# naver-ai/egtr

Measured on AMD Instinct MI355X. Metric: images/sec end-to-end SGG, 600x1000 input, N=200 queries, higher is better.
Workload: dtype f32; 1 GPU; VG inference: ResNet-50, N=200, 6 enc/6 dec, 150 classes, 50 predicates, 600x1000, bs=1/GPU fp32 (BASELINE configs[1]); hip_graph=True, gemm_tuning=True, miopen_find=True, parallelism=replicas x1 (independent images, no collective)

## Files before the change

egtr_amd/_lib.py:

```python
import ctypes
import os

import torch

_HERE = os.path.dirname(os.path.abspath(__file__))
LIB_PATH = os.environ.get("EGTR_HIP_LIBRARY") or os.path.join(_HERE, "libegtr_hip.so")

_P = ctypes.c_void_p
_I = ctypes.c_int
ABI_VERSION = 5

SIGNATURES = {
    "egtr_abi_version": [],
    "egtr_status_string": [_I],
    "egtr_last_hip_error": [],
    "egtr_msda_forward_f32": [_P, _P, _P, _P, _P, _P, _I, _I, _I, _I, _I, _I, _I, _P],
    "egtr_msda_forward_fused_vbias_f32": [_P, _P, _P, _P, _P, _P, _P, _I, _I, _I, _I, _I, _I, _I, _P, _P, _I, _I, _P, _P,
                                          _P],
    "egtr_msda_forward_fused_box_f32": [_P, _P, _P, _P, _P, _P, _P, _I, _I, _I, _I, _I, _I, _I, _P, _P, _I, _I, _P, _P,
                                        _P],
    "egtr_msda_backward_f32": [_P, _P, _P, _P, _P, _P, _P, _I, _I, _I, _I, _I, _I, _I, _P, _P, _P],
    "egtr_msda_backward_out_f32": [_P, _P, _P, _P, _P, _P, _P, _I, _I, _I, _I, _I, _I, _I, _P, _P, _P],
    "egtr_msda_forward_f64": [_P, _P, _P, _P, _P, _P, _I, _I, _I, _I, _I, _I, _I, _P],
    "egtr_msda_backward_f64": [_P, _P, _P, _P, _P, _P, _P, _I, _I, _I, _I, _I, _I, _I, _P, _P, _P],
# ... 18 lines not shown
    "egtr_bias_act_nhwc_bf16": [_P, _P, _P, _P, _P, ctypes.c_longlong, _I, _I],
    "egtr_bias_act_nhwc_f32": [_P, _P, _P, _P, _P, ctypes.c_longlong, _I, _I],
    "egtr_add_layernorm_bf16": [_P, _P, _P, _P, _P, _P, _I, _I, ctypes.c_float],
    "egtr_add_layernorm_pos_bf16": [_P, _P, _P, _P, _P, _P, _I, _I, ctypes.c_float, _P, _I, _P],
    "egtr_add_layernorm_f32": [_P, _P, _P, _P, _P, _P, _I, _I, ctypes.c_float],
    "egtr_sine_pos_embed_f32": [_P, _P, _P, _P, _P, _I, _I, _I, _I, ctypes.c_float, ctypes.c_float],
    "egtr_level_geometry_f32": [_P, _P, _I, _P, _P, _P, _I, _I, _I, _I, _I, ctypes.c_float, ctypes.c_float, _P, _P, _P,
                                _P, _P],
    "egtr_level_geometry_bf16": [_P, _P, _I, _P, _P, _P, _I, _I, _I, _I, _I, ctypes.c_float, ctypes.c_float, _P, _P, _P,
                                 _P, _P],
    "egtr_input_proj_groupnorm_flatten_f32": [_P, _I, _P, _P, _P, _P, _P, _I, _I, _I, ctypes.c_float, _P, _P],
    "egtr_input_proj_groupnorm_flatten_bf16": [_P, _I, _P, _P, _P, _P, _P, _I, _I, _I, ctypes.c_float, _P, _P],
    "egtr_input_proj_groupnorm_tokens_bf16": [_P, _I, _P, _P, _P, _P, _P, _I, _I, _I, ctypes.c_float, _P, _P],
    "egtr_input_proj_groupnorm_tokens_f32": [_P, _I, _P, _P, _P, _P, _P, _I, _I, _I, ctypes.c_float, _P, _P],
    "egtr_input_proj_groupnorm_tokens_workspace_floats": [_I, _P, _I],
    "egtr_bbox_overlaps_f64": [_P, _P, _P, _I, _I, _I, _P],
    "egtr_sgg_eval_width": [_I, _I],
    "egtr_sgg_eval_f32": [_P, _P, _I, _P, _P, _P, _I, _I, _I, _I, _P, _P, ctypes.c_longlong, _P, _P, _P, ctypes.c_longlong,
                          _P, _I, ctypes.c_double, _P, _P, _P],
    "egtr_sgg_zero_shot_f64": [_P, _P, _P, _P, ctypes.c_longlong, _P, _P, ctypes.c_longlong, _I, _I, _I, _I, _P, _P, _I, _P,
                               _P],
    "egtr_sgg_eval_phrdet_f32": [_P, _P, _I, _P, _P, _P, _I, _I, _I, _I, _P, _P, ctypes.c_longlong, _P, _P, _P,
                                 ctypes.c_longlong, _P, _I, ctypes.c_double, _P, _P, _P],
    "egtr_sgg_eval_preddet_f32": [_P, _P, _P, _I, _I, _I, _P, _P, ctypes.c_longlong, _P, ctypes.c_longlong, _P, _I, _P, _P,
                                  _P, _P, _P],
    "egtr_matched_topk_workspace_bytes": [_I, _I, _I],
    "egtr_matched_topk_f32": [_P, _P, _P, _P, _P, _I, _I, _I, _I, _I, _I, _P, _P, _P, _P, _P],
    "egtr_rel_stats_i64": [_P, _P, _P, ctypes.c_longlong, _P, _P, ctypes.c_longlong, _I, _I, _I, _P, _P],
    "egtr_rel_seen_bits_i64": [_P, _P, ctypes.c_longlong, _P],
    "egtr_oi_eval_width": [_I, _I],
# ... 66 lines not shown
    "egtr_proj_ln_x6_f32": [_P, _P, _I, _P, _P, _P, _I, _P, _P, ctypes.c_float, _P, _I, _P, _P, _I, _I],
    "egtr_proj_multi_x6_f32": [_P, _P, _I, _P, _P, _P, _I, _I, _I],
    "egtr_xs_bytes": [_I, _I],
    "egtr_xs_split_f32": [_P, _P, _I, _P, _I, _I, _I, _P, _P, _I],
    "egtr_rel_head_forward_bf16x6_f32": [_P] * 16 + [_I] * 6 + [_P] * 3 + [_I],
    "egtr_rel_head_forward_bf16x6_save_f32": [_P] * 16 + [_I] * 6 + [_P] * 5,
    "egtr_rel_head_streams_f32": [_P] * 4 + [_I] * 2 + [_P] * 3,
    "egtr_rel_head_forward_save_f32": [_P] * 16 + [_I] * 6 + [_P] * 5,
    "egtr_rel_head_backward_pairs_f32": [_P] * 6 + [_I] * 4 + [_P] * 5,
    "egtr_decoder_layer_f32": [_P, _P],
    "egtr_decoder_layer_workspace": [_I, _I, _P, _P, _P],
}
_RESTYPES = {"egtr_status_string": ctypes.c_char_p, "egtr_last_hip_error": ctypes.c_char_p,
             "egtr_ffn_packed_weights_bytes": ctypes.c_longlong,
             "egtr_input_proj_groupnorm_tokens_workspace_floats": ctypes.c_longlong,
             "egtr_msda_backward_bf16_workspace_floats": ctypes.c_longlong,
             "egtr_hungarian_match_scratch_doubles": ctypes.c_longlong,
             "egtr_relation_loss_workspace_bytes": ctypes.c_longlong,
             "egtr_column_sum_workspace_floats": ctypes.c_longlong,
             "egtr_add_layernorm_backward_workspace_floats": ctypes.c_longlong,
             "egtr_linear_split_bf16_wgrad_workspace_floats": ctypes.c_longlong,
             "egtr_dropout_add_layernorm_backward_workspace_floats": ctypes.c_longlong,
             "egtr_xs_bytes": ctypes.c_longlong, "egtr_sgg_eval_width": ctypes.c_longlong,
             "egtr_oi_eval_width": ctypes.c_longlong, "egtr_matched_topk_workspace_bytes": ctypes.c_longlong, "egtr_oi_select_workspace_bytes": ctypes.c_longlong}

_lib = None


class EgtrHipError(RuntimeError):
    pass
# ... 72 lines not shown
```

egtr_amd/csrc/elementwise.hip:

```cpp
#include <hip/hip_runtime.h>
#include <stdint.h>

#include "common.h"

namespace {

__global__ __launch_bounds__(256) void bias_act_nchw_vec4(const float* __restrict__ x, const float* __restrict__ bias,
                                                          const float* __restrict__ res, float* __restrict__ y,
                                                          long long n4, int C, int HW4, int relu) {
  for (long long i = blockIdx.x * (long long)blockDim.x + threadIdx.x; i < n4; i += (long long)gridDim.x * blockDim.x) {
    const int c = (int)((i / HW4) % C);
    const float b = bias[c];
    float4 v = reinterpret_cast<const float4*>(x)[i];
    v.x += b; v.y += b; v.z += b; v.w += b;
    if (res != nullptr) {
      const float4 r = reinterpret_cast<const float4*>(res)[i];
      v.x += r.x; v.y += r.y; v.z += r.z; v.w += r.w;
    }
    if (relu) { v.x = egtr_relu(v.x); v.y = egtr_relu(v.y); v.z = egtr_relu(v.z); v.w = egtr_relu(v.w); }
    reinterpret_cast<float4*>(y)[i] = v;
  }
}

__global__ __launch_bounds__(256) void bias_act_nchw_flat4(const float* __restrict__ x, const float* __restrict__ bias,
// ... 753 lines not shown
  const float* beta[4];
  int hw[4], start[4];
  long long chunk0[5];
  int cchunk0[5];
};

namespace {
__device__ __forceinline__ void load_group8(const unsigned short* x, size_t idx, float (&f)[8]) {
  unpack8(reinterpret_cast<const uint4*>(x)[idx], f);
}
__device__ __forceinline__ void load_group8(const float* x, size_t idx, float (&f)[8]) {
  const float4 a = reinterpret_cast<const float4*>(x)[2 * idx], b = reinterpret_cast<const float4*>(x)[2 * idx + 1];
  f[0] = a.x; f[1] = a.y; f[2] = a.z; f[3] = a.w; f[4] = b.x; f[5] = b.y; f[6] = b.z; f[7] = b.w;
}
constexpr int kGnTokChunk = 256;
template <typename T>
__global__ __launch_bounds__(256) void gn_partial_tokens(GnTokLevels P, int L, int chunks_total, double2* __restrict__ partial) {
  __shared__ double s_red[2][32][9];
  const int b = blockIdx.y;
  int l = 0;
  while (l + 1 < L && (int)blockIdx.x >= P.cchunk0[l + 1]) ++l;
  const int t_begin = ((int)blockIdx.x - P.cchunk0[l]) * kGnTokChunk, hw = P.hw[l];
  const int g = threadIdx.x & 31, ph = threadIdx.x >> 5;
  const T* x = static_cast<const T*>(P.x[l]) + (size_t)b * hw * 256;
  const float4 ba = *reinterpret_cast<const float4*>(P.conv_bias[l] + 8 * g), bb = *reinterpret_cast<const float4*>(P.conv_bias[l] + 8 * g + 4);
  const float cb[8] = {ba.x, ba.y, ba.z, ba.w, bb.x, bb.y, bb.z, bb.w};
  float s1 = 0.f, s2 = 0.f;
#pragma unroll
  for (int u0 = 0; u0 < kGnTokChunk / 8; u0 += 8) {
    float f[8][8];
#pragma unroll
    for (int u = 0; u < 8; ++u) {
      const int t = t_begin + ph + 8 * (u0 + u);
      if (t < hw) load_group8(x, (size_t)t * 32 + g, f[u]);
    }
#pragma unroll
    for (int u = 0; u < 8; ++u) {
      const int t = t_begin + ph + 8 * (u0 + u);
      if (t < hw) {
#pragma unroll
        for (int k = 0; k < 8; ++k) {
          const float v = f[u][k] + cb[k];
          s1 += v;
          s2 += v * v;
        }
      }
    }
  }
  s_red[0][g][ph] = (double)s1;
  s_red[1][g][ph] = (double)s2;
  __syncthreads();
  if (threadIdx.x < 32) {
    double t1 = 0.0, t2 = 0.0;
    for (int w = 0; w < 8; ++w) {
      t1 += s_red[0][threadIdx.x][w];
      t2 += s_red[1][threadIdx.x][w];
    }
    partial[((size_t)b * chunks_total + blockIdx.x) * 32 + threadIdx.x] = make_double2(t1, t2);
  }
// ... 53 lines not shown
#pragma unroll
    for (int k = 0; k < 4; ++k) {
      bf16x2 pr;
      pr[0] = (__bf16)o[2 * k];
      pr[1] = (__bf16)o[2 * k + 1];
      w[k] = __builtin_bit_cast(unsigned, pr);
    }
    reinterpret_cast<uint4*>(dst)[rel] = make_uint4(w[0], w[1], w[2], w[3]);
  } else {
    reinterpret_cast<float4*>(dst)[2 * rel] = make_float4(o[0], o[1], o[2], o[3]);
    reinterpret_cast<float4*>(dst)[2 * rel + 1] = make_float4(o[4], o[5], o[6], o[7]);
  }
}
}

static int gn_tokens_chunks(int num_levels, const int* level_tokens) {
  int c = 0;
  for (int l = 0; l < num_levels; ++l) c += (level_tokens[l] + kGnTokChunk - 1) / kGnTokChunk;
  return c;
}

extern "C" long long egtr_input_proj_groupnorm_tokens_workspace_floats(int num_levels, const int* level_tokens, int batch) {
  if (!level_tokens || num_levels < 1 || num_levels > 4 || batch <= 0) return 0;
  return (long long)num_levels * batch * 64 + (long long)batch * gn_tokens_chunks(num_levels, level_tokens) * 128;
}

static int groupnorm_tokens_launch(egtr_stream_t stream, int num_levels, const void* const* x, const float* const* conv_bias,
                                   const float* const* gamma, const float* const* beta, const int* level_tokens, int batch,
                                   int channels, int num_groups, float eps, float* stats, void* out, bool bf16) {
  if (!x || !conv_bias || !gamma || !beta || !level_tokens || !stats || !out) return EGTR_E_ARG;
  if (num_levels < 1 || num_levels > 4 || batch <= 0) return EGTR_E_ARG;
  if (channels != 256 || num_groups != 32) return EGTR_E_UNSUPPORTED;
  GnTokLevels P;
  int S = 0, cc = 0;
  for (int l = 0; l < 4; ++l) {
    const int s = l < num_levels ? l : 0;
    if (!x[s] || !conv_bias[s] || !gamma[s] || !beta[s] || level_tokens[s] <= 0) return EGTR_E_ARG;
    if (reinterpret_cast<uintptr_t>(x[s]) & 15) return EGTR_E_UNSUPPORTED;
    P.x[l] = x[s];
    P.conv_bias[l] = conv_bias[s];
    P.gamma[l] = gamma[s];
    P.beta[l] = beta[s];
    P.hw[l] = level_tokens[s];
    P.start[l] = S;
    P.chunk0[l] = (long long)S * 32;
    P.cchunk0[l] = cc;
    if (l < num_levels) {
      S += P.hw[l];
      cc += (P.hw[l] + kGnTokChunk - 1) / kGnTokChunk;
    }
  }
  P.chunk0[4] = (long long)S * 32;
  P.cchunk0[4] = cc;
  for (int l = num_levels; l < 4; ++l) {
    P.chunk0[l] = (long long)S * 32;
    P.cchunk0[l] = cc;
  }
  if ((reinterpret_cast<uintptr_t>(out) | reinterpret_cast<uintptr_t>(stats)) & 15) return EGTR_E_UNSUPPORTED;
  hipStream_t st = static_cast<hipStream_t>(stream);
  float2* st2 = reinterpret_cast<float2*>(stats);
  double2* partial = reinterpret_cast<double2*>(stats + (size_t)num_levels * batch * 64);
  const long long chunks = (long long)S * 32;
  const dim3 agrid((unsigned)((chunks + 255) / 256), batch);
  if (bf16) {
    hipLaunchKernelGGL(gn_partial_tokens<unsigned short>, dim3(cc, batch), dim3(256), 0, st, P, num_levels, cc, partial);
    hipLaunchKernelGGL(gn_finalize_tokens, dim3(batch, num_levels), dim3(256), 0, st, P, cc, eps, partial, st2);
    hipLaunchKernelGGL(gn_apply_tokens<unsigned short>, agrid, dim3(256), 0, st, P, num_levels, S, st2,
                       static_cast<unsigned short*>(out));
  } else {
    hipLaunchKernelGGL(gn_partial_tokens<float>, dim3(cc, batch), dim3(256), 0, st, P, num_levels, cc, partial);
    hipLaunchKernelGGL(gn_finalize_tokens, dim3(batch, num_levels), dim3(256), 0, st, P, cc, eps, partial, st2);
    hipLaunchKernelGGL(gn_apply_tokens<float>, agrid, dim3(256), 0, st, P, num_levels, S, st2, static_cast<float*>(out));
  }
  return egtr_check_launch();
}

extern "C" int egtr_input_proj_groupnorm_tokens_bf16(egtr_stream_t stream, int num_levels, const uint16_t* const* x,
                                                     const float* const* conv_bias, const float* const* gamma,
                                                     const float* const* beta, const int* level_tokens, int batch,
                                                     int channels, int num_groups, float eps, float* stats, uint16_t* out) {
  return groupnorm_tokens_launch(stream, num_levels, reinterpret_cast<const void* const*>(x), conv_bias, gamma, beta,
                                 level_tokens, batch, channels, num_groups, eps, stats, out, true);
}

extern "C" int egtr_input_proj_groupnorm_tokens_f32(egtr_stream_t stream, int num_levels, const float* const* x,
                                                    const float* const* conv_bias, const float* const* gamma,
                                                    const float* const* beta, const int* level_tokens, int batch,
                                                    int channels, int num_groups, float eps, float* stats, float* out) {
  return groupnorm_tokens_launch(stream, num_levels, reinterpret_cast<const void* const*>(x), conv_bias, gamma, beta,
                                 level_tokens, batch, channels, num_groups, eps, stats, out, false);
}

extern "C" int egtr_input_proj_groupnorm_flatten_f32(egtr_stream_t stream, int num_levels, const float* const* x,
                                                     const float* const* conv_bias, const float* const* gamma,
                                                     const float* const* beta, const int* level_hw, int batch,
                                                     int channels, int num_groups, float eps, float* stats,
                                                     float* out) {
  return groupnorm_flatten_launch(stream, num_levels, reinterpret_cast<const void* const*>(x), conv_bias, gamma, beta,
                                  level_hw, batch, channels, num_groups, eps, stats, out, false);
}

extern "C" int egtr_input_proj_groupnorm_flatten_bf16(egtr_stream_t stream, int num_levels, const uint16_t* const* x,
                                                      const float* const* conv_bias, const float* const* gamma,
                                                      const float* const* beta, const int* level_hw, int batch,
                                                      int channels, int num_groups, float eps, float* stats,
// ... 502 lines not shown
```

egtr_amd/deformable_detr.py:

```python
import copy
import math
import warnings
from dataclasses import dataclass
from typing import Dict, List, Optional, Tuple

import torch
import torch.nn.functional as F
from torch import Tensor, nn

from . import decoder_fused, ops
from .backbone import DeformableDetrFrozenBatchNorm2d, ResNet50Features, conv1x1_as_gemm
from .hf_compat import ModelOutput, PretrainedConfig, PreTrainedModel
from .ops import MultiScaleDeformableAttentionFunction
from .util import center_to_corners_format, generalized_box_iou, sigmoid_focal_loss

try:
    from scipy.optimize import linear_sum_assignment
except Exception:
    linear_sum_assignment = None

ACT2FN = {"relu": F.relu, "gelu": F.gelu, "silu": F.silu, "tanh": torch.tanh}


class DeformableDetrConfig(PretrainedConfig):
# ... 1147 lines not shown
            conv_encoder = self.backbone.conv_encoder
            if isinstance(conv_encoder, DeformableDetrTimmConvEncoder):
                feature_maps = conv_encoder.model(pixel_values)
            else:
                feature_maps = [fm for fm, _ in conv_encoder(pixel_values, pixel_mask)]
            n_extra = self.config.num_feature_levels - len(feature_maps)
            channels_last = all(fm.dim() == 4 and fm.dtype == pixel_values.dtype and not fm.is_contiguous()
                                and fm.is_contiguous(memory_format=torch.channels_last) for fm in feature_maps)
            if (channels_last and n_extra <= 1 and self.config.d_model == 256
                    and self.input_proj[0][0].weight.dtype == pixel_values.dtype
                    and all(isinstance(p[1], nn.GroupNorm) and p[1].num_groups == 32 and p[0].bias is not None
                            and p[0].groups == 1 for p in self.input_proj)
                    and all(tuple(self.input_proj[l][0].kernel_size) == (1, 1) and tuple(self.input_proj[l][0].stride) == (1, 1)
                            and tuple(self.input_proj[l][0].padding) == (0, 0) for l in range(len(feature_maps)))):
                toks, spatial_shapes_list = [], []
                for level, fm in enumerate(feature_maps):
                    c = self.input_proj[level][0]
                    b_, c_, h_, w_ = fm.shape
                    toks.append(torch.mm(fm.permute(0, 2, 3, 1).reshape(-1, c_), c.weight.detach().view(c.weight.shape[0], c_).t())
                                .view(b_, h_ * w_, -1))
                    spatial_shapes_list.append((h_, w_))
                if n_extra == 1:
                    c = self.input_proj[len(feature_maps)][0]
                    wcl = ops.cached_weights(c, "weight_channels_last", [c.weight],
                                             lambda: c.weight.detach().contiguous(memory_format=torch.channels_last))
                    y = F.conv2d(feature_maps[-1], wcl, None, c.stride, c.padding)
                    toks.append(y.permute(0, 2, 3, 1).reshape(y.shape[0], y.shape[2] * y.shape[3], y.shape[1]))
                    spatial_shapes_list.append(tuple(y.shape[-2:]))
                source_flatten = ops.input_proj_groupnorm_tokens(toks, self.input_proj)
            elif (n_extra <= 1 and self.config.d_model == 256 and feature_maps[0].dtype == pixel_values.dtype
                    and self.input_proj[0][0].weight.dtype == pixel_values.dtype
                    and all(isinstance(p[1], nn.GroupNorm) and p[0].bias is not None for p in self.input_proj)):
                convs = []
                for level, fm in enumerate(feature_maps):
                    c = self.input_proj[level][0]
                    if (tuple(c.kernel_size) == (1, 1) and tuple(c.stride) == (1, 1) and tuple(c.padding) == (0, 0)
                            and c.groups == 1):
                        convs.append(conv1x1_as_gemm(fm, c.weight.detach()))
                    else:
                        convs.append(F.conv2d(fm, c.weight, None, c.stride, c.padding))
                if n_extra == 1:
                    c = self.input_proj[len(feature_maps)][0]
                    convs.append(F.conv2d(feature_maps[-1], c.weight, None, c.stride, c.padding))
                spatial_shapes_list = [tuple(cv.shape[-2:]) for cv in convs]
# ... 522 lines not shown
```

egtr_amd/kernels/backbone.py:

```python
import torch

from .. import _lib
from .._lib import _chk

__all__ = ["bias_relu_maxpool", "xs_bytes", "xs_split", "conv1x1_tail", "stem_weights", "stem_weights_bf16", "stem_fused_bf16",
           "stem_fused", "conv3x3_weights", "conv3x3", "conv1x1_strided", "conv_tail_pack_bf16", "conv1x1_tail_bf16",
           "bias_act_rows_", "bias_act_"]


def bias_relu_maxpool(x, bias):
    N, C, H, W_ = x.shape
    x2 = _chk(x.contiguous(), "x", torch.float32)
    b2 = _chk(bias.contiguous(), "bias", torch.float32)
    y = torch.empty(N, C, (H - 1) // 2 + 1, (W_ - 1) // 2 + 1, dtype=torch.float32, device=x.device)
    _lib.launch("egtr_bias_relu_maxpool3x3s2_f32", x2.data_ptr(), b2.data_ptr(), y.data_ptr(), N, C, H, W_)
    return y


def xs_bytes(rows, K):
    return int(_lib.lib().egtr_xs_bytes(int(rows), int(K)))


def xs_split(x, pos=None, weights=False, plain=True):
    K = x.shape[-1]
# ... 131 lines not shown
    if x.dtype == torch.bfloat16:
        _chk(x, "x", torch.bfloat16)
        _chk(bias, "bias", torch.float32)
        if residual is not None:
            _chk(residual, "residual", torch.bfloat16)
        _lib.launch("egtr_bias_act_nchw_bf16", x.data_ptr(), bias.data_ptr(), _lib.ptr(residual), x.data_ptr(), N, C, H * W_,
                    1 if relu else 0)
        return x
    _chk(x, "x", torch.float32)
    _chk(bias, "bias", torch.float32)
    if residual is not None:
        _chk(residual, "residual", torch.float32)
    _lib.launch("egtr_bias_act_nchw_f32", x.data_ptr(), bias.data_ptr(), _lib.ptr(residual), x.data_ptr(), N, C, H * W_,
                1 if relu else 0)
    return x
```

egtr_amd/kernels/elementwise.py:

```python
import torch

from .. import _lib
from .._lib import _chk
from .derived import cached_weights

__all__ = ["dropout_add_layernorm", "dropout_add_layernorm_backward", "add_layer_norm_into", "box_decode", "bias_mask_rows_",
           "add_layer_norm_pos", "scale_rows_multi", "sine_position_embedding", "input_proj_groupnorm_flatten",
           "input_proj_groupnorm_tokens", "level_geometry"]


def dropout_add_layernorm(x, residual, keep, scale, weight, bias, eps, flag=None):
    rows = x.shape[0]
    y = torch.empty_like(x)
    _lib.launch("egtr_dropout_add_layernorm_f32", x.data_ptr(), residual.data_ptr(), _lib.ptr(keep), float(scale),
                weight.data_ptr(), bias.data_ptr(), y.data_ptr(), rows, 256, float(eps), _lib.ptr(flag))
    return y


def dropout_add_layernorm_backward(x, residual, keep, scale, weight, eps, grad_y, flag=None, y_out=None, clamp_value=0.0):
    lib = _lib.lib()
    rows = x.shape[0]
    gs = torch.empty_like(x)
    gx = torch.empty_like(x) if keep is not None else None
    ws = torch.empty(int(lib.egtr_dropout_add_layernorm_backward_workspace_floats(rows)), dtype=torch.float32, device=x.device)
# ... 174 lines not shown
        if gn.num_groups != 32 or gn.eps != gn0.eps or conv.bias is None or x.shape[-1] != 256 or x.shape[0] != B:
            raise ValueError("input_proj_groupnorm_tokens: 256 channels in 32 groups, one GroupNorm configuration")
    srcs = [t for proj in input_projs[:L] for t in (proj[0].bias, proj[1].weight, proj[1].bias)]
    flat = cached_weights(input_projs, "gn_params_f32", srcs, lambda: [t.detach().float().contiguous() for t in srcs])
    keep = [tuple(flat[3 * l:3 * l + 3]) for l in range(L)]
    toks = [int(x.shape[1]) for x in xs]
    S = sum(toks)
    out = torch.empty(B, S, 256, dtype=dt, device=xs[0].device)
    PA, IA = ctypes.c_void_p * L, ctypes.c_int * L
    stats = torch.empty(int(lib.egtr_input_proj_groupnorm_tokens_workspace_floats(L, IA(*toks), B)), dtype=torch.float32,
                        device=xs[0].device)
    entry = "egtr_input_proj_groupnorm_tokens_bf16" if dt == torch.bfloat16 else "egtr_input_proj_groupnorm_tokens_f32"
    _lib.launch(entry, L, PA(*[x.data_ptr() for x in xs]), PA(*[k[0].data_ptr() for k in keep]),
                PA(*[k[1].data_ptr() for k in keep]), PA(*[k[2].data_ptr() for k in keep]), IA(*toks), B, 256, 32,
                float(gn0.eps), stats.data_ptr(), out.data_ptr())
    return out


_DIM_T = {}


def level_geometry(pixel_mask, spatial_shapes_list, level_embed, embedding_dim, temperature, scale, eps=1e-6):
    import ctypes
    dev = pixel_mask.device
    key = (embedding_dim, float(temperature), str(dev))
    dim_t = _DIM_T.get(key)
    if dim_t is None:
        dim_t = torch.arange(embedding_dim, dtype=torch.float32, device=dev)
        dim_t = temperature ** (2 * torch.div(dim_t, 2, rounding_mode="trunc") / embedding_dim)
        _DIM_T[key] = dim_t
# ... 23 lines not shown
```

egtr_amd/ops.py:

```python
import os

import torch
from torch.autograd import Function
from torch.autograd.function import once_differentiable

from . import _lib
from . import targets as rel_targets
from ._lib import _chk, _stream
from .kernels.backbone import *
from .kernels.derived import *
from .kernels.elementwise import *
from .kernels.elementwise import _DIM_T
from .kernels.heads import *
from .kernels.linear import *
from .kernels.linear import _c16, _host_array, _skinny_bwd, _skinny_fwd, _split3_bf16, _wgrad_ex
from .kernels.protocols import *
from .kernels.statistics import *
from .kernels.vrd import *
from .load_custom import load_hip_kernels

_MSDA = None


def _msda():
# ... 747 lines not shown

GEMM_SPLIT_BF16 = os.environ.get("EGTR_GEMM_SPLIT_BF16", "1") != "0"
LAZY_POS = True
GEMM_SPLIT_MIN_ROWS = 4096
GEMM_SPLIT_WGRAD = True


def gemm_split_supported(x, N, K):
    rows = x.numel() // x.shape[-1]
    eligible = (GEMM_SPLIT_BF16 and x.is_cuda and x.dtype == torch.float32 and not torch.is_grad_enabled()
                and rows >= GEMM_SPLIT_MIN_ROWS)
    return _gate("gemm_split", eligible, eligible and K % 32 == 0 and N % 128 == 0,
                 lambda: f"{rows} x {K} -> {N}: K must be a multiple of 32 and N of 128 (vendor GEMM instead)")


def conv1x1_tail_supported(a, N):
    return (a.is_cuda and a.dtype == torch.float32 and a.dim() == 2 and a.stride(1) == 1 and a.stride(0) % 4 == 0
            and a.data_ptr() % 16 == 0 and a.shape[1] in (64, 128, 256, 512) and N % 64 == 0)


def stem_fused_bf16_supported(x, w):
    return (x.is_cuda and x.dtype == torch.bfloat16 and x.dim() == 4 and x.shape[1] == 3 and x.is_contiguous()
            and tuple(w.shape) == (64, 3, 7, 7) and w.dtype == torch.bfloat16)


def stem_fused_supported(x, w):
    return (x.is_cuda and x.dtype == torch.float32 and x.dim() == 4 and x.shape[1] == 3 and x.is_contiguous()
            and tuple(w.shape) == (64, 3, 7, 7))


# ... 475 lines not shown
```

include/egtr_hip.h:

```cpp
#ifndef EGTR_HIP_H
#define EGTR_HIP_H

#include <stdint.h>

#ifdef __cplusplus
extern "C" {
#endif

typedef void* egtr_stream_t;

enum {
  EGTR_OK = 0,
  EGTR_E_ARG = -1,
  EGTR_E_LAUNCH = -2,
  EGTR_E_UNSUPPORTED = -3
};

#define EGTR_ABI_VERSION 5
int egtr_abi_version(void);
const char* egtr_status_string(int status);
const char* egtr_last_hip_error(void);

int egtr_msda_forward_f32(egtr_stream_t stream, const float* value, const int64_t* spatial_shapes,
                          const int64_t* level_start_index, const float* sampling_loc, const float* attn_weight,
// ... 307 lines not shown
int egtr_input_proj_groupnorm_flatten_bf16(egtr_stream_t stream, int num_levels, const uint16_t* const* x,
                                           const float* const* conv_bias, const float* const* gamma,
                                           const float* const* beta, const int* level_hw, int batch, int channels,
                                           int num_groups, float eps, float* stats, uint16_t* out);

long long egtr_input_proj_groupnorm_tokens_workspace_floats(int num_levels, const int* level_tokens, int batch);
int egtr_input_proj_groupnorm_tokens_bf16(egtr_stream_t stream, int num_levels, const uint16_t* const* x,
                                          const float* const* conv_bias, const float* const* gamma,
                                          const float* const* beta, const int* level_tokens, int batch, int channels,
                                          int num_groups, float eps, float* stats, uint16_t* out);
int egtr_input_proj_groupnorm_tokens_f32(egtr_stream_t stream, int num_levels, const float* const* x,
                                         const float* const* conv_bias, const float* const* gamma, const float* const* beta,
                                         const int* level_tokens, int batch, int channels, int num_groups, float eps,
                                         float* stats, float* out);

int egtr_rel_head_forward_save_f32(egtr_stream_t stream, const float* gate_q, const float* gate_k, const float* uq,
                                   const float* uk, const float* b1, const float* w2r, const float* b2r,
                                   const float* w3r, const float* b3r, const float* w2c, const float* b2c,
                                   const float* w3c, const float* b3c, const float* triplet_dist,
                                   const int64_t* node_cls, int batch, int num_query, int num_slots, int hidden,
                                   int num_rel, int num_cls_plus1, float* rel_logits, float* conn_logits,
                                   float* gate_mean, float* h1_save, float* h2_save);

int egtr_rel_head_forward_bf16w(egtr_stream_t stream, const float* gate_q, const float* gate_k, const float* uq,
                                const float* uk, const float* b1, const uint16_t* w2r, const float* b2r,
                                const uint16_t* w3r, const float* b3r, const uint16_t* w2c, const float* b2c,
                                const uint16_t* w3c, const float* b3c, const float* triplet_dist,
                                const int64_t* node_cls, int batch, int num_query, int num_slots, int hidden,
                                int num_rel, int num_cls_plus1, float* rel_logits, float* conn_logits,
                                float* gate_mean);
// ... 167 lines not shown
```

Measured before the change: 402.4 images/sec.

## Batch all input-projection levels into one split-K bf16x3 MFMA kernel with slab-reducing GroupNorm

Adds one kernel that computes every level's input projection (the 1x1 projections plus the extra 3x3 stride-2 conv done as an implicit GEMM) in a single launch. It uses a three-way bf16 split of fp32 operands on 32x32x16 MFMAs and splits K across blocks, writing partial results into per-split slabs. The GroupNorm partial-stats kernel gains a mode that sums those slabs in place before taking statistics, so no separate split-K reduction kernel is needed. The aim is to replace several vendor GEMM/conv calls and their launches; in exchange there are extra slab memory passes and a more complex split-K plan.

```diff
diff --git a/egtr_amd/_lib.py b/egtr_amd/_lib.py
--- a/egtr_amd/_lib.py
+++ b/egtr_amd/_lib.py
@@ -56,6 +56,10 @@
     "egtr_input_proj_groupnorm_tokens_bf16": [_P, _I, _P, _P, _P, _P, _P, _I, _I, _I, ctypes.c_float, _P, _P],
     "egtr_input_proj_groupnorm_tokens_f32": [_P, _I, _P, _P, _P, _P, _P, _I, _I, _I, ctypes.c_float, _P, _P],
     "egtr_input_proj_groupnorm_tokens_workspace_floats": [_I, _P, _I],
+    "egtr_input_proj_x6_workspace_floats": [_I, _P, _P, _P, _P],
+    "egtr_input_proj_x6_f32": [_P, _I, _P, _P, _P, _P, _P, _P, _P, _I],
+    "egtr_input_proj_groupnorm_token_slabs_workspace_floats": [_I, _P, _P, _I],
+    "egtr_input_proj_groupnorm_token_slabs_f32": [_P, _I, _P, _P, _P, _P, _P, _P, _I, _I, _I, ctypes.c_float, _P, _P],
     "egtr_bbox_overlaps_f64": [_P, _P, _P, _I, _I, _I, _P],
     "egtr_sgg_eval_width": [_I, _I],
     "egtr_sgg_eval_f32": [_P, _P, _I, _P, _P, _P, _I, _I, _I, _I, _P, _P, ctypes.c_longlong, _P, _P, _P, ctypes.c_longlong,
@@ -152,6 +156,8 @@
 _RESTYPES = {"egtr_status_string": ctypes.c_char_p, "egtr_last_hip_error": ctypes.c_char_p,
              "egtr_ffn_packed_weights_bytes": ctypes.c_longlong,
              "egtr_input_proj_groupnorm_tokens_workspace_floats": ctypes.c_longlong,
+             "egtr_input_proj_x6_workspace_floats": ctypes.c_longlong,
+             "egtr_input_proj_groupnorm_token_slabs_workspace_floats": ctypes.c_longlong,
              "egtr_msda_backward_bf16_workspace_floats": ctypes.c_longlong,
              "egtr_hungarian_match_scratch_doubles": ctypes.c_longlong,
              "egtr_relation_loss_workspace_bytes": ctypes.c_longlong,
diff --git a/egtr_amd/csrc/elementwise.hip b/egtr_amd/csrc/elementwise.hip
--- a/egtr_amd/csrc/elementwise.hip
+++ b/egtr_amd/csrc/elementwise.hip
@@ -791,35 +791,81 @@
   f[0] = a.x; f[1] = a.y; f[2] = a.z; f[3] = a.w; f[4] = b.x; f[5] = b.y; f[6] = b.z; f[7] = b.w;
 }
 constexpr int kGnTokChunk = 256;
-template <typename T>
-__global__ __launch_bounds__(256) void gn_partial_tokens(GnTokLevels P, int L, int chunks_total, double2* __restrict__ partial) {
+struct GnTokSlabs {
+  int S[4], ctok[4];
+  long long stride[4];
+};
+__host__ __device__ inline int gn_slab_chunk_tokens(int S) { return S <= 1 ? 256 : S <= 8 ? 32 : S <= 16 ? 16 : 8; }
+template <typename T, bool SPLIT = false>
+__global__ __launch_bounds__(256) void gn_partial_tokens(GnTokLevels P, int L, int chunks_total, double2* __restrict__ partial,
+                                                         GnTokSlabs SL = GnTokSlabs{}) {
   __shared__ double s_red[2][32][9];
   const int b = blockIdx.y;
   int l = 0;
   while (l + 1 < L && (int)blockIdx.x >= P.cchunk0[l + 1]) ++l;
-  const int t_begin = ((int)blockIdx.x - P.cchunk0[l]) * kGnTokChunk, hw = P.hw[l];
+  const int hw = P.hw[l];
   const int g = threadIdx.x & 31, ph = threadIdx.x >> 5;
   const T* x = static_cast<const T*>(P.x[l]) + (size_t)b * hw * 256;
   const float4 ba = *reinterpret_cast<const float4*>(P.conv_bias[l] + 8 * g), bb = *reinterpret_cast<const float4*>(P.conv_bias[l] + 8 * g + 4);
   const float cb[8] = {ba.x, ba.y, ba.z, ba.w, bb.x, bb.y, bb.z, bb.w};
   float s1 = 0.f, s2 = 0.f;
-#pragma unroll
-  for (int u0 = 0; u0 < kGnTokChunk / 8; u0 += 8) {
-    float f[8][8];
-#pragma unroll
-    for (int u = 0; u < 8; ++u) {
-      const int t = t_begin + ph + 8 * (u0 + u);
-      if (t < hw) load_group8(x, (size_t)t * 32 + g, f[u]);
-    }
-#pragma unroll
-    for (int u = 0; u < 8; ++u) {
-      const int t = t_begin + ph + 8 * (u0 + u);
-      if (t < hw) {
+  bool summed = false;
+  if constexpr (SPLIT) {
+    const int ns = SL.S[l];
+    if (ns > 1) {
+      summed = true;
+      const int ct = SL.ctok[l], t0 = ((int)blockIdx.x - P.cchunk0[l]) * ct;
+      const size_t stride = (size_t)SL.stride[l];
+      for (int j = 0; j < ct / 8; ++j) {
+        const int t = t0 + ph + 8 * j;
+        if (t >= hw) break;
+        const size_t idx = (size_t)t * 32 + g;
+        float f[8];
+        load_group8(x, idx, f);
+        for (int sl0 = 1; sl0 < ns; sl0 += 8) {
+          float h[8][8];
+#pragma unroll
+          for (int q = 0; q < 8; ++q)
+            if (sl0 + q < ns) load_group8(x + (size_t)(sl0 + q) * stride, idx, h[q]);
+#pragma unroll
+          for (int q = 0; q < 8; ++q)
+            if (sl0 + q < ns) {
+#pragma unroll
+              for (int k = 0; k < 8; ++k) f[k] += h[q][k];
+            }
+        }
+        float4* dst = reinterpret_cast<float4*>(const_cast<T*>(x)) + 2 * idx;
+        dst[0] = make_float4(f[0], f[1], f[2], f[3]);
+        dst[1] = make_float4(f[4], f[5], f[6], f[7]);
 #pragma unroll
         for (int k = 0; k < 8; ++k) {
-          const float v = f[u][k] + cb[k];
+          const float v = f[k] + cb[k];
           s1 += v;
           s2 += v * v;
+        }
+      }
+    }
+  }
+  if (!summed) {
+    const int t_begin = ((int)blockIdx.x - P.cchunk0[l]) * kGnTokChunk;
+#pragma unroll
+    for (int u0 = 0; u0 < kGnTokChunk / 8; u0 += 8) {
+      float f[8][8];
+#pragma unroll
+      for (int u = 0; u < 8; ++u) {
+        const int t = t_begin + ph + 8 * (u0 + u);
+        if (t < hw) load_group8(x, (size_t)t * 32 + g, f[u]);
+      }
+#pragma unroll
+      for (int u = 0; u < 8; ++u) {
+        const int t = t_begin + ph + 8 * (u0 + u);
+        if (t < hw) {
+#pragma unroll
+          for (int k = 0; k < 8; ++k) {
+            const float v = f[u][k] + cb[k];
+            s1 += v;
+            s2 += v * v;
+          }
         }
       }
     }
@@ -903,9 +949,12 @@
 }
 }
 
-static int gn_tokens_chunks(int num_levels, const int* level_tokens) {
+static int gn_tokens_chunks(int num_levels, const int* level_tokens, const int* splits = nullptr) {
   int c = 0;
-  for (int l = 0; l < num_levels; ++l) c += (level_tokens[l] + kGnTokChunk - 1) / kGnTokChunk;
+  for (int l = 0; l < num_levels; ++l) {
+    const int ct = splits ? gn_slab_chunk_tokens(splits[l]) : kGnTokChunk;
+    c += (level_tokens[l] + ct - 1) / ct;
+  }
   return c;
 }
 
@@ -916,7 +965,8 @@
 
 static int groupnorm_tokens_launch(egtr_stream_t stream, int num_levels, const void* const* x, const float* const* conv_bias,
                                    const float* const* gamma, const float* const* beta, const int* level_tokens, int batch,
-                                   int channels, int num_groups, float eps, float* stats, void* out, bool bf16) {
+                                   int channels, int num_groups, float eps, float* stats, void* out, bool bf16,
+                                   const int* splits = nullptr) {
   if (!x || !conv_bias || !gamma || !beta || !level_tokens || !stats || !out) return EGTR_E_ARG;
   if (num_levels < 1 || num_levels > 4 || batch <= 0) return EGTR_E_ARG;
   if (channels != 256 || num_groups != 32) return EGTR_E_UNSUPPORTED;
@@ -935,8 +985,9 @@
     P.chunk0[l] = (long long)S * 32;
     P.cchunk0[l] = cc;
     if (l < num_levels) {
+      const int ct = splits ? gn_slab_chunk_tokens(splits[l]) : kGnTokChunk;
       S += P.hw[l];
-      cc += (P.hw[l] + kGnTokChunk - 1) / kGnTokChunk;
+      cc += (P.hw[l] + ct - 1) / ct;
     }
   }
   P.chunk0[4] = (long long)S * 32;
@@ -952,12 +1003,24 @@
   const long long chunks = (long long)S * 32;
   const dim3 agrid((unsigned)((chunks + 255) / 256), batch);
   if (bf16) {
-    hipLaunchKernelGGL(gn_partial_tokens<unsigned short>, dim3(cc, batch), dim3(256), 0, st, P, num_levels, cc, partial);
+    hipLaunchKernelGGL(gn_partial_tokens<unsigned short>, dim3(cc, batch), dim3(256), 0, st, P, num_levels, cc, partial,
+                       GnTokSlabs{});
     hipLaunchKernelGGL(gn_finalize_tokens, dim3(batch, num_levels), dim3(256), 0, st, P, cc, eps, partial, st2);
     hipLaunchKernelGGL(gn_apply_tokens<unsigned short>, agrid, dim3(256), 0, st, P, num_levels, S, st2,
                        static_cast<unsigned short*>(out));
+  } else if (splits != nullptr) {
+    GnTokSlabs SL = {};
+    for (int l = 0; l < num_levels; ++l) {
+      if (splits[l] < 1) return EGTR_E_ARG;
+      SL.S[l] = splits[l];
+      SL.ctok[l] = gn_slab_chunk_tokens(splits[l]);
+      SL.stride[l] = (long long)batch * level_tokens[l] * 256;
+    }
+    hipLaunchKernelGGL((gn_partial_tokens<float, true>), dim3(cc, batch), dim3(256), 0, st, P, num_levels, cc, partial, SL);
+    hipLaunchKernelGGL(gn_finalize_tokens, dim3(batch, num_levels), dim3(256), 0, st, P, cc, eps, partial, st2);
+    hipLaunchKernelGGL(gn_apply_tokens<float>, agrid, dim3(256), 0, st, P, num_levels, S, st2, static_cast<float*>(out));
   } else {
-    hipLaunchKernelGGL(gn_partial_tokens<float>, dim3(cc, batch), dim3(256), 0, st, P, num_levels, cc, partial);
+    hipLaunchKernelGGL(gn_partial_tokens<float>, dim3(cc, batch), dim3(256), 0, st, P, num_levels, cc, partial, GnTokSlabs{});
     hipLaunchKernelGGL(gn_finalize_tokens, dim3(batch, num_levels), dim3(256), 0, st, P, cc, eps, partial, st2);
     hipLaunchKernelGGL(gn_apply_tokens<float>, agrid, dim3(256), 0, st, P, num_levels, S, st2, static_cast<float*>(out));
   }
@@ -978,6 +1041,24 @@
                                                     int channels, int num_groups, float eps, float* stats, float* out) {
   return groupnorm_tokens_launch(stream, num_levels, reinterpret_cast<const void* const*>(x), conv_bias, gamma, beta,
                                  level_tokens, batch, channels, num_groups, eps, stats, out, false);
+}
+
+extern "C" long long egtr_input_proj_groupnorm_token_slabs_workspace_floats(int num_levels, const int* level_tokens,
+                                                                            const int* splits, int batch) {
+  if (!level_tokens || !splits || num_levels < 1 || num_levels > 4 || batch <= 0) return 0;
+  for (int l = 0; l < num_levels; ++l)
+    if (splits[l] < 1 || level_tokens[l] <= 0) return 0;
+  return (long long)num_levels * batch * 64 + (long long)batch * gn_tokens_chunks(num_levels, level_tokens, splits) * 128;
+}
+
+extern "C" int egtr_input_proj_groupnorm_token_slabs_f32(egtr_stream_t stream, int num_levels, float* const* slabs,
+                                                         const int* splits, const float* const* conv_bias,
+                                                         const float* const* gamma, const float* const* beta,
+                                                         const int* level_tokens, int batch, int channels, int num_groups,
+                                                         float eps, float* stats, float* out) {
+  if (!splits) return EGTR_E_ARG;
+  return groupnorm_tokens_launch(stream, num_levels, reinterpret_cast<const void* const*>(slabs), conv_bias, gamma, beta,
+                                 level_tokens, batch, channels, num_groups, eps, stats, out, false, splits);
 }
 
 extern "C" int egtr_input_proj_groupnorm_flatten_f32(egtr_stream_t stream, int num_levels, const float* const* x,
diff --git a/egtr_amd/csrc/input_proj_x6.hip b/egtr_amd/csrc/input_proj_x6.hip
--- /dev/null
+++ b/egtr_amd/csrc/input_proj_x6.hip
@@ -0,0 +1,256 @@
+#include <hip/hip_runtime.h>
+#include <stdint.h>
+
+#include "common.h"
+#include "xs_format.h"
+
+namespace {
+
+typedef float f32x16 __attribute__((ext_vector_type(16)));
+typedef float f32x4v __attribute__((ext_vector_type(4)));
+typedef __bf16 bf16x8 __attribute__((ext_vector_type(8)));
+
+constexpr int kBM = 64, kBN = 128, kBK = 32, kN = 256;
+constexpr int kPitch = 40;
+constexpr int kMaxLevels = 4;
+constexpr int kMaxPiece = 512;
+constexpr int kSlots = 512;
+
+__device__ __forceinline__ f32x16 mfma_bf16(bf16x8 a, bf16x8 b, f32x16 c) {
+  return __builtin_amdgcn_mfma_f32_32x32x16_bf16(a, b, c, 0, 0, 0);
+}
+__device__ __forceinline__ f32x4v gload(const void* p) {
+  f32x4v v;
+  asm volatile("global_load_dwordx4 %0, %1, off" : "=&v"(v) : "v"(p));
+  return v;
+}
+__device__ __forceinline__ void vm_wait0(f32x4v& v) { asm volatile("s_waitcnt vmcnt(0)" : "+v"(v)); }
+
+struct IpLevel {
+  const float* A;
+  const unsigned short* Wt;
+  float* ws;
+  int M, K, S, stages;
+  int C, H, W, Ho, Wo;
+  int unit0;
+};
+struct IpLevels {
+  IpLevel p[kMaxLevels];
+};
+
+__device__ __forceinline__ int paired_unit(int bid) {
+  const int x = bid & 7, i = bid >> 3;
+  return 2 * ((i >> 1) * 8 + x) + (i & 1);
+}
+
+__global__ __launch_bounds__(512) __attribute__((amdgpu_waves_per_eu(4, 4))) void input_proj_x6_kernel(IpLevels P, int nlev,
+                                                                                                       int units) {
+  int u = paired_unit(blockIdx.x);
+  if (u >= units) return;
+  int l = 0;
+  while (l + 1 < nlev && u >= P.p[l + 1].unit0) ++l;
+  const IpLevel& G = P.p[l];
+  u -= G.unit0;
+  const int mblocks = (G.M + kBM - 1) / kBM;
+  const int nb = u & 1, mt = (u >> 1) % mblocks, ks = (u >> 1) / mblocks;
+  const int m0 = mt * kBM, M = G.M, nstage = G.stages, stage0 = ks * nstage;
+  const float* __restrict__ A = G.A;
+  const bool conv = G.C != 0;
+
+  constexpr int kStageElems = 3 * kBM * kPitch + 3 * kBN * kPitch;
+  __shared__ __attribute__((aligned(16))) __bf16 sbase[kStageElems];
+  __bf16* sA = sbase;
+  __bf16* sW = sbase + 3 * kBM * kPitch;
+  const int tid = threadIdx.x, lane = tid & 63, wave = tid >> 6;
+  const int wm = wave >> 2, wn = wave & 3;
+  const int li = lane & 31, hf = lane >> 5;
+
+  const int lrow = tid >> 3, c4 = tid & 7;
+  const int row = min(m0 + lrow, M - 1);
+  const float* aplain = A + (size_t)row * G.K + 4 * c4;
+  int iy0 = 0, ix0 = 0;
+  const float* aimg = A;
+  if (conv) {
+    const int hw = G.Ho * G.Wo, b = row / hw, r = row - b * hw, y = r / G.Wo, x = r - y * G.Wo;
+    iy0 = 2 * y - 1;
+    ix0 = 2 * x - 1;
+    aimg = A + (size_t)b * G.H * G.W * G.C + 4 * c4;
+  }
+  const char* wblk = reinterpret_cast<const char*>(G.Wt) + (size_t)nb * (G.K / kBK) * (3 * kBN * kBK * 2) + (size_t)tid * 16;
+
+  f32x4v ra, rw[3];
+  bool live = true;
+  auto issue = [&](int s) {
+    const int st = stage0 + s;
+    const float* ap;
+    if (conv) {
+      const int k = st * kBK, tap = k / G.C, c0 = k - tap * G.C, dy = tap / 3, dx = tap - 3 * dy;
+      const int iy = iy0 + dy, ix = ix0 + dx;
+      live = iy >= 0 && iy < G.H && ix >= 0 && ix < G.W;
+      ap = live ? aimg + ((size_t)iy * G.W + ix) * G.C + c0 : aimg;
+    } else {
+      ap = aplain + (size_t)st * kBK;
+    }
+    ra = gload(ap);
+    const char* wp = wblk + (size_t)st * (3 * kBN * kBK * 2);
+#pragma unroll
+    for (int q = 0; q < 3; ++q) rw[q] = gload(wp + q * 8192);
+  };
+  auto stash = [&]() {
+    vm_wait0(ra);
+#pragma unroll
+    for (int q = 0; q < 3; ++q) vm_wait0(rw[q]);
+    if (!live) ra = f32x4v{0.f, 0.f, 0.f, 0.f};
+    {
+      const xs::Split3 s0 = xs::split3_fast(ra.x), s1 = xs::split3_fast(ra.y), s2 = xs::split3_fast(ra.z),
+                       s3 = xs::split3_fast(ra.w);
+      __bf16* p = sA + lrow * kPitch + 4 * c4;
+      *reinterpret_cast<uint2*>(p) = make_uint2(xs::pack_hi16(s0.hi, s1.hi), xs::pack_hi16(s2.hi, s3.hi));
+      *reinterpret_cast<uint2*>(p + kBM * kPitch) = make_uint2(xs::pack_hi16(s0.mid, s1.mid), xs::pack_hi16(s2.mid, s3.mid));
+      *reinterpret_cast<uint2*>(p + 2 * kBM * kPitch) = make_uint2(xs::pack_hi16(s0.lo, s1.lo), xs::pack_hi16(s2.lo, s3.lo));
+    }
+#pragma unroll
+    for (int q = 0; q < 3; ++q) {
+      const int idx = tid + 512 * q;
+      const int piece = idx >> 9, wr = (idx >> 2) & 127, c = idx & 3;
+      *reinterpret_cast<f32x4v*>(sW + (piece * kBN + wr) * kPitch + 8 * c) = rw[q];
+    }
+  };
+
+  f32x16 acc, acc_hi;
+#pragma unroll
+  for (int r = 0; r < 16; ++r) acc[r] = acc_hi[r] = 0.f;
+
+  issue(0);
+  stash();
+  __syncthreads();
+  const __bf16* pa0 = sA + (wm * 32 + li) * kPitch + 8 * hf;
+  const __bf16* pw0 = sW + (wn * 32 + li) * kPitch + 8 * hf;
+  auto compute = [&]() {
+#pragma unroll
+    for (int k2 = 0; k2 < 2; ++k2) {
+      bf16x8 a[3], w[3];
+#pragma unroll
+      for (int p = 0; p < 3; ++p) {
+        a[p] = *reinterpret_cast<const bf16x8*>(pa0 + p * kBM * kPitch + 16 * k2);
+        w[p] = *reinterpret_cast<const bf16x8*>(pw0 + p * kBN * kPitch + 16 * k2);
+      }
+      f32x16 c = acc;
+      c = mfma_bf16(w[2], a[0], c);
+      c = mfma_bf16(w[0], a[2], c);
+      c = mfma_bf16(w[1], a[1], c);
+      c = mfma_bf16(w[1], a[0], c);
+      c = mfma_bf16(w[0], a[1], c);
+      acc = c;
+      acc_hi = mfma_bf16(w[0], a[0], acc_hi);
+    }
+  };
+#pragma unroll 1
+  for (int s = 0; s + 1 < nstage; ++s) {
+    issue(s + 1);
+    compute();
+    __syncthreads();
+    stash();
+    __syncthreads();
+  }
+  compute();
+#pragma unroll
+  for (int r = 0; r < 16; ++r) acc[r] += acc_hi[r];
+
+  const int orow = m0 + wm * 32 + li;
+  if (orow < M) {
+    float* out = G.ws + ((size_t)ks * M + orow) * kN + nb * kBN + wn * 32 + 4 * hf;
+#pragma unroll
+    for (int q = 0; q < 4; ++q)
+      *reinterpret_cast<float4*>(out + 8 * q) = make_float4(acc[4 * q + 0], acc[4 * q + 1], acc[4 * q + 2], acc[4 * q + 3]);
+  }
+}
+
+struct IpPlan {
+  int S[kMaxLevels];
+  long long floats;
+  long long units;
+};
+bool plan_levels(int n, const int* rows, const int* K, const int* tapc, IpPlan* out) {
+  if (n < 1 || n > kMaxLevels || !rows || !K) return false;
+  int piece[kMaxLevels];
+  long long tiles[kMaxLevels], units = 0;
+  for (int l = 0; l < n; ++l) {
+    const int unit_k = (tapc && tapc[l]) ? tapc[l] : K[l];
+    if (rows[l] <= 0 || K[l] <= 0 || unit_k % kBK || K[l] % unit_k) return false;
+    int d = std::min(unit_k, kMaxPiece) / kBK * kBK;
+    while (unit_k % d) d -= kBK;
+    piece[l] = d;
+    tiles[l] = 2LL * ((rows[l] + kBM - 1) / kBM);
+    units += tiles[l] * (K[l] / d);
+  }
+  for (bool again = true; again;) {
+    again = false;
+    for (int l = 0; l < n; ++l) {
+      const long long own = tiles[l] * (K[l] / piece[l]);
+      if (own >= kSlots || piece[l] % (2 * kBK) || units + own > 2 * kSlots) continue;
+      piece[l] /= 2;
+      units += own;
+      again = true;
+    }
+  }
+  out->floats = 0;
+  out->units = units;
+  for (int l = 0; l < n; ++l) {
+    out->S[l] = K[l] / piece[l];
+    out->floats += (long long)out->S[l] * rows[l] * kN;
+  }
+  return true;
+}
+
+}
+
+extern "C" long long egtr_input_proj_x6_workspace_floats(int num_levels, const int* rows, const int* K, const int* tap_channels,
+                                                         int* splits) {
+  IpPlan pl;
+  if (!splits || !plan_levels(num_levels, rows, K, tap_channels, &pl)) return 0;
+  for (int l = 0; l < num_levels; ++l) splits[l] = pl.S[l];
+  return pl.floats;
+}
+
+extern "C" int egtr_input_proj_x6_f32(egtr_stream_t stream, int num_levels, const float* const* x,
+                                      const uint16_t* const* w_tiled, float* const* workspace, const int* rows, const int* K,
+                                      const int* conv_geometry, const int* splits, int N) {
+  if (!x || !w_tiled || !workspace || !rows || !K || !splits || num_levels < 1) return EGTR_E_ARG;
+  if (num_levels > kMaxLevels || N != kN) return EGTR_E_UNSUPPORTED;
+  IpLevels P = {};
+  long long units = 0;
+  for (int l = 0; l < num_levels; ++l) {
+    if (!x[l] || !w_tiled[l] || !workspace[l] || rows[l] <= 0 || K[l] <= 0 || splits[l] <= 0) return EGTR_E_ARG;
+    const int* g = conv_geometry ? conv_geometry + 4 * l : nullptr;
+    IpLevel& L = P.p[l];
+    if (g && g[3] != 0) {
+      if (g[0] <= 0 || g[1] <= 0 || g[2] <= 0 || g[3] < 0) return EGTR_E_ARG;
+      L.H = g[1];
+      L.W = g[2];
+      L.C = g[3];
+      L.Ho = (g[1] - 1) / 2 + 1;
+      L.Wo = (g[2] - 1) / 2 + 1;
+      if ((long long)g[0] * L.Ho * L.Wo != rows[l] || 9LL * L.C != K[l]) return EGTR_E_ARG;
+      if (L.C % kBK) return EGTR_E_UNSUPPORTED;
+    }
+    if (K[l] % kBK || (reinterpret_cast<uintptr_t>(x[l]) & 15) || (reinterpret_cast<uintptr_t>(w_tiled[l]) & 15) ||
+        (reinterpret_cast<uintptr_t>(workspace[l]) & 15) || (long long)rows[l] * K[l] >= (1LL << 40))
+      return EGTR_E_UNSUPPORTED;
+    if ((K[l] / kBK) % splits[l]) return EGTR_E_ARG;
+    L.A = x[l];
+    L.Wt = reinterpret_cast<const unsigned short*>(w_tiled[l]);
+    L.ws = workspace[l];
+    L.M = rows[l];
+    L.K = K[l];
+    L.S = splits[l];
+    L.stages = K[l] / kBK / splits[l];
+    L.unit0 = (int)units;
+    units += 2LL * ((rows[l] + kBM - 1) / kBM) * splits[l];
+    if (units >= (1LL << 30)) return EGTR_E_UNSUPPORTED;
+  }
+  const unsigned grid = (unsigned)((units + 15) / 16 * 16);
+  hipLaunchKernelGGL(input_proj_x6_kernel, dim3(grid), dim3(512), 0, static_cast<hipStream_t>(stream), P, num_levels,
+                     (int)units);
+  return egtr_check_launch();
+}
diff --git a/egtr_amd/deformable_detr.py b/egtr_amd/deformable_detr.py
--- a/egtr_amd/deformable_detr.py
+++ b/egtr_amd/deformable_detr.py
@@ -1185,20 +1185,25 @@
                     and all(tuple(self.input_proj[l][0].kernel_size) == (1, 1) and tuple(self.input_proj[l][0].stride) == (1, 1)
                             and tuple(self.input_proj[l][0].padding) == (0, 0) for l in range(len(feature_maps)))):
                 toks, spatial_shapes_list = [], []
-                for level, fm in enumerate(feature_maps):
+                grouped = (len(self.input_proj) == len(feature_maps) + n_extra
+                           and ops.input_proj_x6_supported(feature_maps, self.input_proj))
+                if grouped:
+                    source_flatten, spatial_shapes_list = ops.input_proj_x6_groupnorm(feature_maps, self.input_proj)
+                for level, fm in enumerate(feature_maps if not grouped else ()):
                     c = self.input_proj[level][0]
                     b_, c_, h_, w_ = fm.shape
                     toks.append(torch.mm(fm.permute(0, 2, 3, 1).reshape(-1, c_), c.weight.detach().view(c.weight.shape[0], c_).t())
                                 .view(b_, h_ * w_, -1))
                     spatial_shapes_list.append((h_, w_))
-                if n_extra == 1:
+                if n_extra == 1 and not grouped:
                     c = self.input_proj[len(feature_maps)][0]
                     wcl = ops.cached_weights(c, "weight_channels_last", [c.weight],
                                              lambda: c.weight.detach().contiguous(memory_format=torch.channels_last))
                     y = F.conv2d(feature_maps[-1], wcl, None, c.stride, c.padding)
                     toks.append(y.permute(0, 2, 3, 1).reshape(y.shape[0], y.shape[2] * y.shape[3], y.shape[1]))
                     spatial_shapes_list.append(tuple(y.shape[-2:]))
-                source_flatten = ops.input_proj_groupnorm_tokens(toks, self.input_proj)
+                if not grouped:
+                    source_flatten = ops.input_proj_groupnorm_tokens(toks, self.input_proj)
             elif (n_extra <= 1 and self.config.d_model == 256 and feature_maps[0].dtype == pixel_values.dtype
                     and self.input_proj[0][0].weight.dtype == pixel_values.dtype
                     and all(isinstance(p[1], nn.GroupNorm) and p[0].bias is not None for p in self.input_proj)):
diff --git a/egtr_amd/kernels/backbone.py b/egtr_amd/kernels/backbone.py
--- a/egtr_amd/kernels/backbone.py
+++ b/egtr_amd/kernels/backbone.py
@@ -5,7 +5,7 @@
 
 __all__ = ["bias_relu_maxpool", "xs_bytes", "xs_split", "conv1x1_tail", "stem_weights", "stem_weights_bf16", "stem_fused_bf16",
            "stem_fused", "conv3x3_weights", "conv3x3", "conv1x1_strided", "conv_tail_pack_bf16", "conv1x1_tail_bf16",
-           "bias_act_rows_", "bias_act_"]
+           "bias_act_rows_", "bias_act_", "input_proj_x6_plan", "input_proj_x6_weights", "input_proj_x6"]
 
 
 def bias_relu_maxpool(x, bias):
@@ -169,3 +169,65 @@
     _lib.launch("egtr_bias_act_nchw_f32", x.data_ptr(), bias.data_ptr(), _lib.ptr(residual), x.data_ptr(), N, C, H * W_,
                 1 if relu else 0)
     return x
+
+
+def input_proj_x6_plan(rows, K, tap_channels):
+    import ctypes
+    L = len(rows)
+    IA = ctypes.c_int * L
+    splits = IA()
+    n = int(_lib.lib().egtr_input_proj_x6_workspace_floats(L, IA(*[int(v) for v in rows]), IA(*[int(v) for v in K]),
+                                                           IA(*[int(v) for v in tap_channels]), splits))
+    if n <= 0:
+        raise RuntimeError(f"input_proj_x6_plan: rows {list(rows)}, K {list(K)}, tap channels {list(tap_channels)} are not served")
+    return [int(v) for v in splits], n
+
+
+def input_proj_x6_weights(w):
+    w = w.detach()
+    N = w.shape[0]
+    wm = w.permute(0, 2, 3, 1).reshape(N, -1).contiguous()
+    out = torch.empty(N // 128, wm.shape[1] // 32, 3, 128, 32, dtype=torch.bfloat16, device=w.device)
+    _lib.launch("egtr_gemm_split_tile_weights_f32", wm.data_ptr(), wm.stride(0), 0, N, wm.shape[1], out.data_ptr())
+    return out
+
+
+def input_proj_x6(maps, w_tiled, strided3x3, splits=None, slabs=None):
+    import ctypes
+    L = len(maps)
+    if not (L == len(w_tiled) == len(strided3x3)):
+        raise ValueError("input_proj_x6: one weight and one kind per level")
+    B = maps[0].shape[0]
+    rows, Ks, tapc, geom, shapes = [], [], [], [], []
+    for fm, conv in zip(maps, strided3x3):
+        b, c, h, w = fm.shape
+        if (not fm.is_cuda or fm.dtype != torch.float32 or b != B or not fm.is_contiguous(memory_format=torch.channels_last)
+                or fm.data_ptr() % 16):
+            raise RuntimeError("input_proj_x6: channels-last float32 device feature maps, 16-byte aligned")
+        if conv:
+            ho, wo = (h - 1) // 2 + 1, (w - 1) // 2 + 1
+            rows.append(b * ho * wo)
+            Ks.append(9 * c)
+            tapc.append(c)
+            geom += [b, h, w, c]
+            shapes.append((ho, wo))
+        else:
+            rows.append(b * h * w)
+            Ks.append(c)
+            tapc.append(0)
+            geom += [0, 0, 0, 0]
+            shapes.append((h, w))
+    for l in range(L):
+        if w_tiled[l].numel() != 3 * 256 * Ks[l] or w_tiled[l].dtype != torch.bfloat16:
+            raise ValueError(f"input_proj_x6: weight stream {l} is not that of a [256, {Ks[l]}] matrix")
+    plan, _ = input_proj_x6_plan(rows, Ks, tapc)
+    splits = plan if splits is None else [int(v) for v in splits]
+    want = [(splits[l], B, rows[l] // B, 256) for l in range(L)]
+    if slabs is None:
+        slabs = [torch.empty(w, dtype=torch.float32, device=maps[0].device) for w in want]
+    elif [tuple(t.shape) for t in slabs] != want or any(t.dtype != torch.float32 or not t.is_contiguous() for t in slabs):
+        raise ValueError(f"input_proj_x6: slabs must be contiguous float32 tensors of shapes {want}")
+    PA, IA = ctypes.c_void_p * L, ctypes.c_int * L
+    _lib.launch("egtr_input_proj_x6_f32", L, PA(*[x.data_ptr() for x in maps]), PA(*[w.data_ptr() for w in w_tiled]),
+                PA(*[s.data_ptr() for s in slabs]), IA(*rows), IA(*Ks), (ctypes.c_int * (4 * L))(*geom), IA(*splits), 256)
+    return slabs, splits, shapes
diff --git a/egtr_amd/kernels/elementwise.py b/egtr_amd/kernels/elementwise.py
--- a/egtr_amd/kernels/elementwise.py
+++ b/egtr_amd/kernels/elementwise.py
@@ -6,7 +6,7 @@
 
 __all__ = ["dropout_add_layernorm", "dropout_add_layernorm_backward", "add_layer_norm_into", "box_decode", "bias_mask_rows_",
            "add_layer_norm_pos", "scale_rows_multi", "sine_position_embedding", "input_proj_groupnorm_flatten",
-           "input_proj_groupnorm_tokens", "level_geometry"]
+           "input_proj_groupnorm_tokens", "input_proj_groupnorm_token_slabs", "level_geometry"]
 
 
 def dropout_add_layernorm(x, residual, keep, scale, weight, bias, eps, flag=None):
@@ -212,6 +212,31 @@
     _lib.launch(entry, L, PA(*[x.data_ptr() for x in xs]), PA(*[k[0].data_ptr() for k in keep]),
                 PA(*[k[1].data_ptr() for k in keep]), PA(*[k[2].data_ptr() for k in keep]), IA(*toks), B, 256, 32,
                 float(gn0.eps), stats.data_ptr(), out.data_ptr())
+    return out
+
+
+def input_proj_groupnorm_token_slabs(slabs, input_projs):
+    import ctypes
+    lib = _lib.lib()
+    L = len(slabs)
+    B = slabs[0].shape[1]
+    gn0 = input_projs[0][1]
+    xs = [_chk(x, "slabs", torch.float32) for x in slabs]
+    for proj, x in zip(input_projs[:L], xs):
+        conv, gn = proj[0], proj[1]
+        if gn.num_groups != 32 or gn.eps != gn0.eps or conv.bias is None or x.dim() != 4 or x.shape[-1] != 256 or x.shape[1] != B:
+            raise ValueError("input_proj_groupnorm_token_slabs: [S, B, tokens, 256] slabs, 32 groups, one GroupNorm configuration")
+    srcs = [t for proj in input_projs[:L] for t in (proj[0].bias, proj[1].weight, proj[1].bias)]
+    flat = cached_weights(input_projs, "gn_params_f32", srcs, lambda: [t.detach().float().contiguous() for t in srcs])
+    keep = [tuple(flat[3 * l:3 * l + 3]) for l in range(L)]
+    toks = [int(x.shape[2]) for x in xs]
+    out = torch.empty(B, sum(toks), 256, dtype=torch.float32, device=xs[0].device)
+    PA, IA = ctypes.c_void_p * L, ctypes.c_int * L
+    splits = IA(*[int(x.shape[0]) for x in xs])
+    stats = torch.empty(int(lib.egtr_input_proj_groupnorm_token_slabs_workspace_floats(L, IA(*toks), splits, B)),
+                        dtype=torch.float32, device=xs[0].device)
+    _lib.launch("egtr_input_proj_groupnorm_token_slabs_f32", L, PA(*[x.data_ptr() for x in xs]), splits, PA(*[k[0].data_ptr() for k in keep]), PA(*[k[1].data_ptr() for k in keep]),
+                PA(*[k[2].data_ptr() for k in keep]), IA(*toks), B, 256, 32, float(gn0.eps), stats.data_ptr(), out.data_ptr())
     return out
 
 
diff --git a/egtr_amd/ops.py b/egtr_amd/ops.py
--- a/egtr_amd/ops.py
+++ b/egtr_amd/ops.py
@@ -785,6 +785,40 @@
                  lambda: f"{rows} x {K} -> {N}: K must be a multiple of 32 and N of 128 (vendor GEMM instead)")
 
 
+def input_proj_x6_supported(feature_maps, input_proj):
+    maps = list(feature_maps)
+    L = len(input_proj)
+    eligible = (GEMM_SPLIT_BF16 and len(maps) > 0 and not torch.is_grad_enabled()
+                and all(fm.is_cuda and fm.dtype == torch.float32 for fm in maps)
+                and all(p[0].weight.dtype == torch.float32 for p in input_proj))
+    if not eligible:
+        return False
+
+    def conv_ok(c, k, s, p):
+        return (tuple(c.kernel_size) == (k, k) and tuple(c.stride) == (s, s) and tuple(c.padding) == (p, p)
+                and tuple(c.dilation) == (1, 1) and c.groups == 1 and c.out_channels == 256 and c.in_channels % 32 == 0)
+    ok = (len(maps) <= L <= min(len(maps) + 1, 4)
+          and all(fm.dim() == 4 and fm.is_contiguous(memory_format=torch.channels_last) and fm.data_ptr() % 16 == 0
+                  and fm.shape[0] == maps[0].shape[0] for fm in maps)
+          and all(conv_ok(input_proj[l][0], 1, 1, 0) and input_proj[l][0].in_channels == maps[l].shape[1]
+                  for l in range(len(maps)))
+          and (L == len(maps) or (conv_ok(input_proj[L - 1][0], 3, 2, 1)
+                                  and input_proj[L - 1][0].in_channels == maps[-1].shape[1])))
+    return _gate("input_proj_x6", True, ok,
+                 lambda: f"maps {[tuple(fm.shape) for fm in maps]}: channels-last, channels a multiple of 32, 1x1 projections to "
+                         "256 channels and at most one 3x3 / stride 2 extra level are served (vendor products instead)")
+
+
+def input_proj_x6_groupnorm(feature_maps, input_proj):
+    L = len(input_proj)
+    wts = [cached_weights(input_proj[l][0], "input_proj_x6_weights", [input_proj[l][0].weight],
+                          lambda l=l: input_proj_x6_weights(input_proj[l][0].weight)) for l in range(L)]
+    maps = list(feature_maps)
+    extra = L - len(maps)
+    slabs, _, shapes = input_proj_x6(maps + maps[-1:] * extra, wts, [False] * len(maps) + [True] * extra)
+    return input_proj_groupnorm_token_slabs(slabs, input_proj), shapes
+
+
 def conv1x1_tail_supported(a, N):
     return (a.is_cuda and a.dtype == torch.float32 and a.dim() == 2 and a.stride(1) == 1 and a.stride(0) % 4 == 0
             and a.data_ptr() % 16 == 0 and a.shape[1] in (64, 128, 256, 512) and N % 64 == 0)
diff --git a/include/egtr_hip.h b/include/egtr_hip.h
--- a/include/egtr_hip.h
+++ b/include/egtr_hip.h
@@ -345,6 +345,18 @@
                                          const int* level_tokens, int batch, int channels, int num_groups, float eps,
                                          float* stats, float* out);
 
+long long egtr_input_proj_x6_workspace_floats(int num_levels, const int* rows, const int* K, const int* tap_channels,
+                                              int* splits);
+int egtr_input_proj_x6_f32(egtr_stream_t stream, int num_levels, const float* const* x, const uint16_t* const* w_tiled,
+                           float* const* workspace, const int* rows, const int* K, const int* conv_geometry,
+                           const int* splits, int N);
+long long egtr_input_proj_groupnorm_token_slabs_workspace_floats(int num_levels, const int* level_tokens, const int* splits,
+                                                                int batch);
+int egtr_input_proj_groupnorm_token_slabs_f32(egtr_stream_t stream, int num_levels, float* const* slabs, const int* splits,
+                                              const float* const* conv_bias, const float* const* gamma,
+                                              const float* const* beta, const int* level_tokens, int batch, int channels,
+                                              int num_groups, float eps, float* stats, float* out);
+
 int egtr_rel_head_forward_save_f32(egtr_stream_t stream, const float* gate_q, const float* gate_k, const float* uq,
                                    const float* uk, const float* b1, const float* w2r, const float* b2r,
                                    const float* w3r, const float* b3r, const float* w2c, const float* b2c,
```

Result: faster. 406.8 images/sec, median of 6 (+1.1%).
